# xiph/daala

Hardware: AMD Instinct MI355X
Metric: 1080p all-intra transform blocks/s (filter+DCT+PVQ) (higher is better)
Workload: dtype int32 (lifting DCT/filters) + f64 (PVQ search)

## Files before the change

### daala_amd/build.py

```python
import os
import subprocess
import sys
from concurrent.futures import ThreadPoolExecutor

HERE = os.path.dirname(os.path.abspath(__file__))
CSRC = os.path.join(HERE, "csrc")
LIBDIR = os.path.join(HERE, "lib")
LIB = os.path.join(LIBDIR, "libdaalahip.so")
EXP_LIB = os.path.join(LIBDIR, "libdaalahip_exp.so")
EXP_OBJDIR = os.path.join(LIBDIR, "exp")
HIPCC = os.environ.get("HIPCC", "/opt/rocm/bin/hipcc")
SOURCES = ["dct_kernels.hip", "lapped_kernels.hip", "pvq_kernels.hip", "pvq_bands.hip", "pvq_ref.hip", "pvq_refbands.hip", "image_kernels.hip", "dering_kernels.hip", "dering_cache.hip", "frame_cache.hip",
           "odhip_host.hip", "ctx.hip", "quant.hip", "pipeline.hip", "y4m.hip", "dist_kernels.hip", "rate_host.hip", "export_kernels.hip", "metrics_kernels.hip", "mc_kernels.hip"]
FLAGS = ["--offload-arch=gfx950", "-O3", "-std=c++17", "-fPIC",
         "-ffp-contract=off", "-fno-fast-math", "-Wall",
         "-Wno-unused-function"]


def _deps():
    out = []
    for root, _, files in os.walk(CSRC):
        for f in files:
            out.append(os.path.join(root, f))
    out.append(os.path.join(os.path.dirname(HERE), "include", "daala_hip.h"))
    return out


def _stale(target, deps):
    if not os.path.exists(target):
        return True
    t = os.path.getmtime(target)
    return any(os.path.getmtime(d) > t for d in deps)


def build(force=False, verbose=False, experiments=True):
    os.makedirs(LIBDIR, exist_ok=True)
    os.makedirs(EXP_OBJDIR, exist_ok=True)
    deps = _deps()
    variants = [(LIB, LIBDIR, [])]
    if experiments:
        variants.append((EXP_LIB, EXP_OBJDIR, ["-DODHIP_EXPERIMENTS"]))

    def run(cmd):
        if verbose:
            print(" ".join(cmd), flush=True)
        r = subprocess.run(cmd, capture_output=True, text=True)
        if r.returncode != 0:
            raise RuntimeError("hipcc failed:\n%s\n%s" % (" ".join(cmd), r.stderr))
        return r.stderr

    for lib, objdir, extra in variants:
        objs = []
        jobs = []
        for src in SOURCES:
            obj = os.path.join(objdir, src.replace(".hip", ".o"))
            objs.append(obj)
            if force or _stale(obj, deps):
                jobs.append([HIPCC] + FLAGS + extra + ["-c", os.path.join(CSRC, src), "-o", obj])
        try:
            with ThreadPoolExecutor(max_workers=min(8, os.cpu_count() or 4)) as ex:
                for warn in ex.map(run, jobs):
                    if verbose and warn:
                        print(warn)
            if jobs or force or _stale(lib, objs):
                run([HIPCC, "--offload-arch=gfx950", "-shared", "-fPIC", "-o", lib] + objs)
        except RuntimeError:
            if lib == LIB or experiments != "optional":
                raise
            print("daala_amd.build: the experiments variant failed to build (the product library is intact)",
                  file=sys.stderr)
    return LIB


def build_variant(name, extra_flags, verbose=False):
    outdir = os.path.join(HERE, "lib_" + name)
    os.makedirs(outdir, exist_ok=True)
    lib = os.path.join(outdir, "libdaalahip.so")
    stamp = os.path.join(outdir, "flags.txt")
    flags_changed = not os.path.exists(stamp) or open(stamp).read() != " ".join(extra_flags)
    deps = _deps()
    jobs = []
    objs = []
    for src in SOURCES:
        obj = os.path.join(outdir, src.replace(".hip", ".o"))
        objs.append(obj)
        if flags_changed or _stale(obj, deps):
            jobs.append([HIPCC] + FLAGS + list(extra_flags) + ["-c", os.path.join(CSRC, src), "-o", obj])

    def run(cmd):
        if verbose:
            print(" ".join(cmd), flush=True)
        r = subprocess.run(cmd, capture_output=True, text=True)
        if r.returncode != 0:
            raise RuntimeError("hipcc failed:\n%s\n%s" % (" ".join(cmd), r.stderr))

    with ThreadPoolExecutor(max_workers=min(8, os.cpu_count() or 4)) as ex:
        list(ex.map(run, jobs))
    if jobs or not os.path.exists(lib):
        run([HIPCC, "--offload-arch=gfx950", "-shared", "-fPIC", "-o", lib] + objs)
    with open(stamp, "w") as f:
        f.write(" ".join(extra_flags))
    return lib


if __name__ == "__main__":
    if "--variant" in sys.argv:
        i = sys.argv.index("--variant")
        print(build_variant(sys.argv[i + 1], sys.argv[i + 2:], verbose=True))
    else:
        print(build(force="--force" in sys.argv, verbose=True))
```

### daala_amd/csrc/od_sel.cuh

```cuda
#pragma once

namespace {

__device__ __forceinline__ unsigned long long od_cmp_gt(double a, double b) {
  unsigned long long m;
  asm("v_cmp_gt_f64_e64 %0, %1, %2" : "=s"(m) : "v"(a), "v"(b));
  return m;
}

__device__ __forceinline__ int od_sel(unsigned long long m, int t, int f) {
  int d;
  asm("v_cndmask_b32_e64 %0, %1, %2, %3" : "=v"(d) : "v"(f), "v"(t), "s"(m));
  return d;
}

__device__ __forceinline__ void od_inc(int &j) {
  asm("v_add_u32 %0, 1, %0" : "+v"(j));
}

__device__ __forceinline__ double od_cvt_u(int v) {
  double d;
  asm volatile("v_cvt_f64_u32_e32 %0, %1" : "=v"(d) : "v"(v));
  return d;
}

__device__ __forceinline__ double od_sel(unsigned long long m, double t, double f) {
  const int lo = od_sel(m, __double2loint(t), __double2loint(f));
  const int hi = od_sel(m, __double2hiint(t), __double2hiint(f));
  return __hiloint2double(hi, lo);
}

}
```

### daala_amd/csrc/pvq_refbands.hip

```cpp
#include "../../include/daala_hip.h"
#include <math.h>
#include <stdio.h>
#include <stdlib.h>
#include <string.h>
#include "od_ctx.cuh"
#include "od_pvq_math.cuh"
#include "od_occupancy.cuh"
#include "od_krange.cuh"
#include "od_band_stage.cuh"
#include "gen/od_scan_tables.h"
#define OD_RSQ_TABLE_N 512
#define OD_RSQ_HUGE
#include "pvq_search.cuh"
#include "pvq_row.cuh"
#include "pvq_regs.cuh"

namespace {

constexpr int kMaxJobs = 8;
constexpr int kMaxItems = kMaxJobs*ODHIP_MAX_BANDS;
constexpr int kSlots = ODHIP_PVQ_REF_SLOTS;
constexpr int kUncCap = 1 << 16;
constexpr double kDefaultMargin = 1e-9;

// ... 673 lines not shown
      int32_t tmp = odq_mult16_16(r16[e], proj_1);
      tmp = outshift >= 0 ? odq_shr_round(tmp, outshift) : odq_shl32(tmp, -outshift);
      const int16_t v = (int16_t)(x16[e] - tmp);
      if (live && i != m) xro[i - (i > m)] = v;
    }
  }
  if (live) {
    if constexpr (E == 8) {
      *reinterpret_cast<uint4 *>(x16o + l*E) = make_uint4(pack16(x16[0], x16[1]),
       pack16(x16[2], x16[3]), pack16(x16[4], x16[5]), pack16(x16[6], x16[7]));
      *reinterpret_cast<uint4 *>(r16o + l*E) = make_uint4(pack16(r16[0], r16[1]),
       pack16(r16[2], r16[3]), pack16(r16[4], r16[5]), pack16(r16[6], r16[7]));
    }
    else {
#pragma unroll
      for (int e = 0; e < E; e += 2) {
        *reinterpret_cast<uint32_t *>(x16o + l*E + e) = pack16(x16[e], x16[e + 1]);
        *reinterpret_cast<uint32_t *>(r16o + l*E + e) = pack16(r16[e], r16[e + 1]);
      }
    }
    if (l == 0) prep_write(it, rec + band, job, band, blk, xshift, rshift, p, r_null, flip, m, s);
  }
}


struct ItemPtr {
  int4 *head;
  int4 *tail;
  int4 *res;
  long stride;
};

__device__ __forceinline__ ItemPtr item_ptr(const RJob &jb, int band, long blk) {
  ItemPtr p;
  const long plane = (long)jb.nb_bands*kSlots*jb.nblocks;
  p.head = reinterpret_cast<int4 *>(jb.items) + (long)band*kSlots*jb.nblocks + blk;
  p.tail = p.head + plane;
  p.res = p.tail + plane;
  p.stride = jb.nblocks;
  return p;
}

__device__ __forceinline__ void refb_candidates(const RJob &jb, int band, long blk,
 int theta_override, int4 (*stage)[kWave]) {
  const int lane = threadIdx.x;
  odhip_pvq_refband *rp = jb.rec + blk*jb.nb_bands + band;
  odhip_pvq_refband r = *rp;
  if (theta_override >= 0) r.theta = theta_override;
  const int n = jb.off[band + 1] - jb.off[band];
  const int beta = jb.beta[band];
  const ItemPtr ip = item_ptr(jb, band, blk);
  int nitems = 0;
  int kmax_theta = 0;
  int kmax_noref = 0;
  if (r.flags & ODHIP_REFBAND_THETA) {
    const int gain_bound = (r.cg - r.gain_offset) >> ODQ_CGAIN_SHIFT;
    const double scale_1 = __ddiv_rn(1., kThetaScale);
    for (int i = gain_bound - 1 > 1 ? gain_bound - 1 : 1; i <= gain_bound + 1; i++) {
      const int32_t qcg = odq_shl32(i, ODQ_CGAIN_SHIFT) + r.gain_offset;
      const int ts = odq_pvq_compute_max_theta(qcg, beta);
      const double t = __ddiv_rn(((r.theta*scale_1)*2), kPi)*ts;
      int lower = (int)floor(.5 + t) - 2;
      if (lower < 0) lower = 0;
      int upper = (int)ceil(t);
      if (upper > ts - 1) upper = ts - 1;
      for (int j = lower; j <= upper && nitems < kSlots - 2; j++) {
        const int4 c = make_int4(i, j, ts, odq_compute_k_ref(j, n));
        kmax_theta = c.w > kmax_theta ? c.w : kmax_theta;
        int pos = nitems;
        while (pos > 0) {
          const int4 q = stage[pos - 1][lane];
          const int cmp = q.w == c.w ? q.x - c.x : q.w - c.w;
          if (cmp <= 0) break;
          stage[pos][lane] = q;
          pos--;
        }
        stage[pos][lane] = c;
        nitems++;
      }
    }
  }
  const int ntheta = nitems;
  int flags = r.flags & ~ODHIP_REFBAND_NOREF;
  if ((jb.is_keyframe && jb.pli == 0) || r.corr < .5 || r.cg < odq_shl32(2, ODQ_CGAIN_SHIFT)) {
    flags |= ODHIP_REFBAND_NOREF;
    const int gain_bound = r.cg >> ODQ_CGAIN_SHIFT;
    for (int i = gain_bound > 1 ? gain_bound : 1; i <= gain_bound + 1; i++) {
      const int kk = odq_compute_k_noref(odq_shl32(i, ODQ_CGAIN_SHIFT), n, beta);
      stage[nitems][lane] = make_int4(i, -1, 0, kk);
      kmax_noref = kk > kmax_noref ? kk : kmax_noref;
      nitems++;
    }
  }
  for (int i = 0; i < nitems; i++) ip.head[i*ip.stride] = stage[i][lane];
  int4 v;
  v.x = (int)((uint32_t)(uint16_t)r.m | (uint32_t)(uint8_t)r.s << 16 | (uint32_t)flags << 24);
  v.y = r.theta;
  v.z = nitems;
  v.w = ntheta;
  reinterpret_cast<int4 *>(rp)[2] = v;
  jb.keys[(long)band*jb.nblocks + blk] = (unsigned short)(kSortBins - 1 - od_work_bin(kmax_theta + kmax_noref));
}

__global__ __launch_bounds__(kWave) void k_refb_cands(RItems it) {
  const int item = find_item(it, blockIdx.x);
  const RJob &jb = it.jobs[it.job[item]];
  const long blk = (long)(blockIdx.x - it.wg_start[item])*kWave + threadIdx.x;
  __shared__ int4 stage[kSlots][kWave];
  if (blk >= jb.nblocks) return;
  refb_candidates(jb, it.band[item], blk, -1, stage);
}

__global__ __launch_bounds__(kWave) void k_refb_cands_list(const RJob *jobs, const Unc *list, int count) {
  __shared__ int4 stage[kSlots][kWave];
  const int i = blockIdx.x*kWave + threadIdx.x;
  if (i >= count) return;
  const Unc e = list[i];
  refb_candidates(jobs[e.job], e.band, e.blk, e.theta, stage);
}

struct RefBest {
  double best_cost;
  int chosen;
  int yslot;
  int noref;
  int32_t qtheta;
  int gain;
  int theta;
  int ts;
  int k;
  bool close;
};

struct NoDecide {
  template <class V>
  __device__ __forceinline__ void offer(int, bool, const int4 &, int32_t, int, double, int, const V &) {}
};

template <class V, class D>
__device__ __forceinline__ void refb_loops(const RJob &jb, int band, long blk, bool writer,
 bool may_store, double lambda, V &v, D &dec) {
  const odhip_pvq_refband r = jb.rec[blk*jb.nb_bands + band];
  const int off = jb.off[band];
  const int n = jb.off[band + 1] - off;
  const long nblocks = jb.nblocks;
  const int len = jb.len;
  int16_t *const yout = jb.y;
  const ItemPtr ip = item_ptr(jb, band, blk);
  const double s2 = (1./256)*(1./256);
  const double t1 = 1./32768;
  const int32_t cg = r.cg;
  const double dist0 = r.dist0;
  if (r.ntheta > 0) {
    v.load(jb.xr + blk*len + off, true);
    int prev_k = 0;
    int cur_slot = -1;
    int cur_mom = 0;
    double cos_dist = 0;
    const int32_t theta = r.theta;
    int4 hnext = ip.head[0];
    for (int idx = 0; idx < r.ntheta; idx++) {
      const int4 h = hnext;
      hnext = ip.head[(idx + 1 < r.nitems ? idx + 1 : idx)*ip.stride];
      const int32_t qcg = odq_shl32(h.x, ODQ_CGAIN_SHIFT) + r.gain_offset;
      const int32_t qtheta = odq_pvq_compute_theta(h.y, h.z);
      const int k = h.w;
      double dist_theta = 2 - (2.*odq_pvq_cos(theta - qtheta))*t1;
      double dist = (1.4*(qcg - cg))*(qcg - cg) + (qcg*(double)cg)*dist_theta;
      dist *= s2;
      if (dist > dist0 + 1.0*lambda && k != 0) {
        if (writer) ip.tail[idx*ip.stride] = make_int4(qcg, qtheta, ODHIP_REFITEM_WITH_REF, -1);
        continue;
      }
      if (k > ODHIP_PVQ_MAX_K) {
        if (writer) {
          atomicAdd(jb.krange, 1u);
          ip.tail[idx*ip.stride] = make_int4(qcg, qtheta, ODHIP_REFITEM_WITH_REF | ODHIP_REFITEM_K_RANGE,
           -1);
        }
        continue;
      }
      const double sin_prod = ((odq_pvq_sin(theta)*t1)*odq_pvq_sin(qtheta))*t1;
      if (k == 0) {
        cos_dist = 0;
        cur_slot = -1;
        cur_mom = 0;
      }
      else if (k != prev_k) {
        cos_dist = v.search(n - 1, k, prev_k, ((qcg*(double)cg)*sin_prod)*s2, lambda);
        cur_slot = idx;
        cur_mom = v.moment();
        if (may_store) v.store(yout + ((long)idx*nblocks + blk)*len + off);
      }
      prev_k = k;
      dist_theta = 2 - (2.*odq_pvq_cos(theta - qtheta))*t1 + sin_prod*(2 - 2*cos_dist);
      dist = (1.4*(qcg - cg))*(qcg - cg) + (qcg*(double)cg)*dist_theta;
      dist *= s2;
      if (writer) {
        ip.tail[idx*ip.stride] = make_int4(qcg, qtheta,
         ODHIP_REFITEM_WITH_REF | ODHIP_REFITEM_SEARCHED | cur_mom << ODHIP_REFITEM_MOMENT_SHIFT, cur_slot);
        ip.res[idx*ip.stride] = make_int4(__double2loint(cos_dist), __double2hiint(cos_dist),
         __double2loint(dist), __double2hiint(dist));
      }
      dec.offer(idx, true, h, qtheta, cur_slot, dist, cur_mom, v);
    }
  }
  if (r.nitems > r.ntheta) {
    v.load(jb.x16 + blk*len + off, false);
    int prev_k = 0;
    for (int idx = r.ntheta; idx < r.nitems; idx++) {
      const int4 h = ip.head[idx*ip.stride];
      const int32_t qcg = odq_shl32(h.x, ODQ_CGAIN_SHIFT);
      const int k = h.w;
      double dist = (1.4*(qcg - cg))*(qcg - cg);
      dist *= s2;
      if (dist > dist0 && k != 0) {
        if (writer) ip.tail[idx*ip.stride] = make_int4(qcg, 0, 0, -1);
        continue;
      }
      if (k > ODHIP_PVQ_MAX_K) {
        if (writer) atomicAdd(jb.krange, 1u);
        if (writer) ip.tail[idx*ip.stride] = make_int4(qcg, 0, ODHIP_REFITEM_K_RANGE, -1);
        continue;
      }
      const double cos_dist = v.search(n, k, prev_k, (qcg*(double)cg)*s2, lambda);
      prev_k = k;
      const int mom = v.moment();
      if (may_store) v.store(yout + ((long)idx*nblocks + blk)*len + off);
      dist = (1.4*(qcg - cg))*(qcg - cg) + (qcg*(double)cg)*(2 - 2*cos_dist);
      dist *= s2;
      if (writer) {
        ip.tail[idx*ip.stride] = make_int4(qcg, 0, ODHIP_REFITEM_SEARCHED | mom << ODHIP_REFITEM_MOMENT_SHIFT, idx);
        ip.res[idx*ip.stride] = make_int4(__double2loint(cos_dist), __double2hiint(cos_dist),
         __double2loint(dist), __double2hiint(dist));
      }
      dec.offer(idx, false, h, 0, idx, dist, mom, v);
    }
  }
}

struct LdsVector {
  short *xs;
  unsigned short *ys;
  int lane;
  int n;
  __device__ __forceinline__ void load(const int16_t *src, bool pad) {
    const int cnt = n - (pad ? 1 : 0);
    for (int j = 0; j < cnt; j++) xs[j*kWave + lane] = src[j];
  }
  __device__ __forceinline__ double search(int n_true, int k, int prev_k, double g2, double lambda) {
    double yy;
    cur = n_true;
    return od_pvq_search_lane(xs, ys, lane, n_true, k, prev_k, g2, lambda, &yy);
  }
  __device__ __forceinline__ void store(int16_t *dst) {
    for (int j = 0; j < cur; j++) {
      const int yj = ys[j*kWave + lane];
      dst[j] = (int16_t)(xs[j*kWave + lane] < 0 ? -yj : yj);
    }
  }
  __device__ __forceinline__ int moment() const {
    int m = 0;
    for (int j = 1; j < cur; j++) m += j*ys[j*kWave + lane];
    return m;
  }
  int cur;
};

#ifdef ODHIP_EXPERIMENTS
__global__ __launch_bounds__(kWave) void k_refb_search(RItems it) {
  extern __shared__ __attribute__((aligned(16))) unsigned short lds[];
  od_rsqrt_init(threadIdx.x);
  const int item = find_item(it, blockIdx.x);
  const RJob &jb = it.jobs[it.job[item]];
  const int band = it.band[item];
  const int n = jb.off[band + 1] - jb.off[band];
  const long pos = (long)(blockIdx.x - it.wg_start[item])*kWave + threadIdx.x;
  if (pos >= jb.nblocks) return;
  const long blk = jb.ids[(long)band*jb.nblocks + pos];
  LdsVector v = {(short *)lds, lds + n*kWave, (int)threadIdx.x, n, 0};
  NoDecide nd;
  refb_loops(jb, band, blk, true, true, it.lambda, v, nd);
}
#endif

__global__ __launch_bounds__(kWave) void k_refb_search_list(const RJob *jobs, const Unc *list, int count,
 double lambda) {
  extern __shared__ __attribute__((aligned(16))) unsigned short lds[];
  od_rsqrt_init(threadIdx.x);
  if (threadIdx.x != 0 || (int)blockIdx.x >= count) return;
  const Unc e = list[blockIdx.x];
  const RJob &jb = jobs[e.job];
  LdsVector v = {(short *)lds, lds + 128*kWave, 0, jb.off[e.band + 1] - jb.off[e.band], 0};
  NoDecide nd;
  refb_loops(jb, e.band, e.blk, true, true, lambda, v, nd);
}

__device__ __forceinline__ uint32_t pack_pulses(int s0, int y0, int s1, int y1) {
  return pack16(s0 ? -y0 : y0, s1 ? -y1 : y1);
}

template <int E, int G>
struct RowVector {
  int ax[E];
  unsigned sg;
  int y[E];
  int row;
  int l;
  int force;
  double xx;
  double norm_1;
  double cxy;
  double cyy;
  __device__ __forceinline__ void load(const int16_t *src, bool pad) {
    const int16_t *p = src + l*E;
    sg = 0;
#pragma unroll
    for (int e = 0; e < E; e++) {
      const int v = p[e];
      ax[e] = abs(v);
      sg |= (unsigned)(v < 0) << e;
      y[e] = 0;
    }
    if (pad && l == G - 1) {
      ax[E - 1] = 0;
      sg &= ~(1u << (E - 1));
    }
    od_row_norm<E, G>(ax, &xx, &norm_1);
  }
  __device__ __forceinline__ double search(int n_true, int k, int prev_k, double g2, double lambda) {
#ifdef ODHIP_EXPERIMENTS
    const int placed = prev_k > 0 && prev_k <= k ? prev_k : 0;
    const int greedy = k - (1 + k/4) - placed;
    pulses += greedy > 0 ? greedy : 0;
    rate_pulses += k - placed - (greedy > 0 ? greedy : 0);
    return od_pvq_search_row<E, G>(ax, y, row, l, n_true, k, prev_k, g2, lambda, force, xx, norm_1,
     &cxy, &cyy, &replays);
#else
    return od_pvq_search_row<E, G>(ax, y, row, l, n_true, k, prev_k, g2, lambda, force, xx, norm_1,
     &cxy, &cyy);
#endif
  }
#ifdef ODHIP_EXPERIMENTS
  int replays = 0;
  int pulses = 0;
  int rate_pulses = 0;
#endif
  __device__ __forceinline__ int moment() const {
    int m = 0;
#pragma unroll
    for (int e = 0; e < E; e++) m += (l*E + e)*y[e];
    return grp_sum<G>(m);
  }
  __device__ __forceinline__ void store(int16_t *dst) {
    int16_t *p = dst + l*E;
    if constexpr (E == 8) {
      *reinterpret_cast<uint4 *>(p) = make_uint4(pack_pulses(sg & 1, y[0], sg & 2, y[1]),
       pack_pulses(sg & 4, y[2], sg & 8, y[3]), pack_pulses(sg & 16, y[4], sg & 32, y[5]),
       pack_pulses(sg & 64, y[6], sg & 128, y[7]));
    }
    else {
#pragma unroll
      for (int e = 0; e < E; e += 2) {
        *reinterpret_cast<uint32_t *>(p + e) = pack_pulses(sg & (1u << e), y[e], sg & (2u << e), y[e + 1]);
      }
    }
  }
};

#ifdef ODHIP_EXPERIMENTS
__device__ unsigned long long gRowReplayStats[4];
#endif

template <int E, int G>
__global__ __launch_bounds__(kWave) void k_pvq_search_row(const int16_t *x_in, int n_true, const int32_t *k_in,
 od_coeff *y_out, const double *g2_in, double lambda, int force_scan, double *cos_out, int32_t *replays_out,
 long nbands) {
  constexpr int n = E*G;
  constexpr int C = kWave/G;
  od_rsqrt_init(threadIdx.x);
  const int lane = threadIdx.x;
  const int row = lane/G;
  const int l = lane%G;
  const long band = (long)blockIdx.x*C + row;
  const bool live = band < nbands;
  const long b = live ? band : nbands - 1;
  int ax[E];
  int y[E];
  unsigned sg = 0;
#pragma unroll
  for (int e = 0; e < E; e++) {
    const int j = l*E + e;
    const int v = j < n_true ? x_in[b*n_true + j] : 0;
    ax[e] = abs(v);
    sg |= (unsigned)(v < 0) << e;
    y[e] = 0;
  }
  double xx;
  double norm_1;
  od_row_norm<E, G>(ax, &xx, &norm_1);
  double cxy = 0;
  double cyy = 0;
  int replays = 0;
  int k = k_in[b];
  k = k < 0 ? 0 : k > 32767 ? 32767 : k;
  const double c = od_pvq_search_row<E, G>(ax, y, row, l, n_true, k, 0, g2_in[b], lambda, force_scan, xx, norm_1,
   &cxy, &cyy, &replays);
  if (live) {
#pragma unroll
    for (int e = 0; e < E; e++) {
      const int j = l*E + e;
      if (j < n_true) y_out[band*n_true + j] = sg >> e & 1 ? -y[e] : y[e];
    }
    if (l == 0) {
      cos_out[band] = c;
      if (replays_out) replays_out[band] = replays;
    }
  }
  (void)n;
}

template <int E, int G>
__global__ __launch_bounds__(kWave) __attribute__((amdgpu_waves_per_eu(3, 3))) void k_refb_search_row(RItems it) {
  od_rsqrt_init(threadIdx.x);
  const int item = find_item(it, blockIdx.x);
  const RJob &jb = it.jobs[it.job[item]];
  const int lane = threadIdx.x;
  RowVector<E, G> v;
  v.row = lane/G;
  v.l = lane%G;
  v.force = it.perturb >> 1;
  const long nblocks = jb.nblocks;
  const long pos = (long)(blockIdx.x - it.wg_start[item])*(kWave/G) + v.row;
  const bool live = pos < nblocks;
  const long blk = jb.ids[(long)it.band[item]*nblocks + (live ? pos : nblocks - 1)];
  NoDecide nd;
  refb_loops(jb, it.band[item], blk, live && v.l == 0, live, it.lambda, v, nd);
}

template <int N>
struct RegVector {
  static constexpr int SH = N == 15 ? 1 : 0;
  int ax[N];
  unsigned sg;
  int y[N];
  double xx;
  double norm_1;
  double cxy;
  double cyy;
  __device__ __forceinline__ void load(const int16_t *src, bool pad) {
    const uint4 *p = reinterpret_cast<const uint4 *>(src - SH);
    sg = 0;
    uint32_t w[(N + SH)/2];
#pragma unroll
    for (int q = 0; q < (N + SH)/8; q++) {
      const uint4 t = p[q];
      w[4*q] = t.x;
      w[4*q + 1] = t.y;
      w[4*q + 2] = t.z;
      w[4*q + 3] = t.w;
    }
#pragma unroll
    for (int i = 0; i < N; i++) {
      const int t = (int16_t)(w[(i + SH) >> 1] >> (16*((i + SH) & 1)));
      ax[i] = abs(t);
      sg |= (unsigned)(t < 0) << i;
      y[i] = 0;
    }
    if (pad) {
      ax[N - 1] = 0;
      sg &= ~(1u << (N - 1));
    }
    od_regs_norm<N>(ax, &xx, &norm_1);
  }
  __device__ __forceinline__ double search(int n_true, int k, int prev_k, double g2, double lambda) {
    return od_pvq_search_regs<N>(ax, y, n_true, k, prev_k, g2, lambda, xx, norm_1, &cxy, &cyy);
  }
  __device__ __forceinline__ int moment() const {
    int m = 0;
#pragma unroll
    for (int i = 1; i < N; i++) m += i*y[i];
    return m;
  }
  __device__ __forceinline__ void store(int16_t *dst) {
    uint4 *p = reinterpret_cast<uint4 *>(dst - SH);
    int t[N + SH];
    if (SH) t[0] = 0;
#pragma unroll
    for (int i = 0; i < N; i++) t[i + SH] = (sg >> i) & 1 ? -y[i] : y[i];
#pragma unroll
    for (int q = 0; q < (N + SH)/8; q++) {
      p[q] = make_uint4(pack16(t[8*q], t[8*q + 1]), pack16(t[8*q + 2], t[8*q + 3]),
       pack16(t[8*q + 4], t[8*q + 5]), pack16(t[8*q + 6], t[8*q + 7]));
    }
  }
};



__device__ __forceinline__ int neg_interleave(int x, int ref) {
  if (x < ref) return -2*(x - ref) - 1;
  if (x < 2*ref) return 2*(x - ref);
  return x - 1;
}

__device__ unsigned char gRBandOf[OD_SCAN_LEN];

template <int N, class YGet>
__device__ __forceinline__ void refb_finish(const RItems &it, int job, const RJob &jb, int band, long blk,
 const odhip_pvq_refband &r, const RefBest &best, YGet yget);

template <int N, int PRICE>
__device__ __forceinline__ void refb_choose_band(const RItems &it, int job, const RJob &jb, int band,
 long blk, const double *given) {
  constexpr int SH = N == 15 ? 1 : 0;
  constexpr int NW = (N + SH)/2;
  const long bi = blk*jb.nb_bands + band;
  const odhip_pvq_refband r = jb.rec[bi];
  const ItemPtr ip = item_ptr(jb, band, blk);
  const double *rate = PRICE == 2 ? given : PRICE == 0 && jb.rate ? jb.rate + bi*(kSlots + 1) : nullptr;
  const double lambda = it.lambda;
  const int off = jb.off[band];
  double best_cost = r.dist0 + lambda*(rate ? rate[0] : 0.);
  bool close = false;
  int noref = jb.is_keyframe ? 1 : 0;
  int32_t best_qtheta = 0;
  int chosen = -1;
  int yslot = -1;
  int4 tails[kSlots];
  int dlo[kSlots];
  int dhi[kSlots];
#pragma unroll
  for (int idx = 0; idx < kSlots; idx++) {
    tails[idx] = make_int4(0, 0, 0, -1);
    dlo[idx] = 0;
    dhi[idx] = 0;
    if (idx < r.nitems) {
      tails[idx] = ip.tail[idx*ip.stride];
      const int4 res = ip.res[idx*ip.stride];
      dlo[idx] = res.z;
      dhi[idx] = res.w;
    }
  }
#pragma unroll
  for (int idx = 0; idx < kSlots; idx++) {
    if (idx >= r.nitems) continue;
    const int4 tail = tails[idx];
    if (!(tail.z & ODHIP_REFITEM_SEARCHED)) continue;
    double cost = __hiloint2double(dhi[idx], dlo[idx]);
    if (PRICE == 1) {
      const int4 hd = ip.head[idx*ip.stride];
      const bool with_ref = idx < r.ntheta;
      const int sum = (int)((unsigned)tail.z >> ODHIP_REFITEM_MOMENT_SHIFT);
      cost = cost + lambda*odq_pvq_rate_fast(sum, hd.w, N, hd.x, with_ref ? r.icgr : 0, with_ref ? hd.y : -1,
       with_ref ? hd.z : 0, jb.is_keyframe, jb.pli);
      const double d = cost - best_cost;
      if ((d < 0 ? -d : d) <= it.tol_scale*odq_rate_tol(cost, best_cost)) close = true;
    }
    else cost = cost + lambda*(rate ? rate[1 + idx] : 0.);
    if (idx < r.ntheta ? cost < best_cost : cost <= best_cost) {
      best_cost = cost;
      chosen = idx;
      yslot = tail.w;
      if (idx < r.ntheta) {
        best_qtheta = tail.y;
        noref = 0;
      }
      else noref = 1;
    }
  }
  RefBest best;
  best.best_cost = best_cost;
  best.chosen = chosen;
  best.yslot = yslot;
  best.noref = noref;
  best.qtheta = best_qtheta;
  best.gain = best.theta = best.ts = best.k = 0;
  best.close = PRICE == 1 && close;
  if (chosen >= 0) {
    const int4 head = ip.head[chosen*ip.stride];
    best.gain = head.x;
    best.theta = head.y;
    best.ts = head.z;
    best.k = head.w;
  }
  uint32_t yw[NW];
  if (yslot >= 0) {
    const uint4 *yp = reinterpret_cast<const uint4 *>(jb.y + ((long)yslot*jb.nblocks + blk)*jb.len
     + off - SH);
    if constexpr (NW >= 4) {
#pragma unroll
      for (int v = 0; v < NW/4; v++) {
        const uint4 q = yp[v];
        yw[4*v] = q.x;
        yw[4*v + 1] = q.y;
        yw[4*v + 2] = q.z;
        yw[4*v + 3] = q.w;
      }
    }
  }
  else {
#pragma unroll
    for (int v = 0; v < NW; v++) yw[v] = 0;
  }
  refb_finish<N>(it, job, jb, band, blk, r, best,
   [&](int i) -> int { return (int16_t)(yw[(i + SH) >> 1] >> (16*((i + SH) & 1))); });
}

template <int N, class YGet>
__device__ __forceinline__ void refb_finish(const RItems &it, int job, const RJob &jb, int band, long blk,
 const odhip_pvq_refband &r, const RefBest &best, YGet yget) {
  constexpr int SH = N == 15 ? 1 : 0;
  constexpr int NW = (N + SH)/2;
  const long bi = blk*jb.nb_bands + band;
  const int off = jb.off[band];
  const int cfl_enabled = jb.is_keyframe && jb.pli != 0;
  const int chosen = best.chosen;
  const int yslot = best.yslot;
  const int noref = best.noref;
  const int32_t best_qtheta = best.qtheta;
  int qg = 0;
  int itheta = jb.is_keyframe ? -1 : 0;
  int max_theta = 0;
  int best_k = 0;
  if (best.close) {
    const unsigned slot = atomicAdd(it.pcount, 1u);
    if (slot < (unsigned)kPUncCap) {
      PUncR *e = it.plist + slot;
      e->job = job;
      e->band = band;
      e->blk = (unsigned)blk;
    }
  }
  if (chosen >= 0) {
    qg = best.gain;
    best_k = best.k;
    if (noref) {
      itheta = -1;
      max_theta = 0;
    }
    else {
      itheta = best.theta;
      max_theta = best.ts;
    }
  }
  int skip = 0;
  if (noref) {
    if (qg == 0) skip = 1;
  }
  else {
    if (!jb.is_keyframe && qg == 0) skip = r.icgr ? 1 : 2;
    if (qg == r.icgr && itheta == 0 && !cfl_enabled) skip = 2;
  }
  int4 *ch = reinterpret_cast<int4 *>(jb.choice + bi*16);
  ch[0] = make_int4(chosen, qg, noref, itheta);
  ch[1] = make_int4(max_theta, best_k, skip, jb.is_keyframe ? (noref ? qg : neg_interleave(qg, r.icgr))
   : (noref ? qg - 1 : neg_interleave(qg + 1, r.icgr + 1)));
  if (skip) {
    const int flip = (r.flags & ODHIP_REFBAND_FLIP) != 0;
    ch[2] = make_int4(skip == 2 ? (flip ? 4 : 1) : 0, -1, 0, 0);
    ch[3] = make_int4(0, 0, 0, 0);
    return;
  }
  const int32_t g = odq_gain_expand(odq_shl32(qg, ODQ_CGAIN_SHIFT) + (noref ? 0 : r.gain_offset),
   job_q(jb, band, blk), jb.beta[band]);
  const int nn = N - (!noref);
  int yy = 0;
#pragma unroll
  for (int i = 0; i < N; i++) {
    const int v = i < nn ? yget(i) : 0;
    yy += v*v;
  }
  int gshift = odq_ilog(g) - 14;
  gshift = gshift > 0 ? gshift : 0;
  int32_t scale = 0;
  if (yy != 0) {
    int rsqrt_shift;
    const int16_t rsqrt = odq_rsqrt(yy, &rsqrt_shift);
    scale = odq_vshr_round(rsqrt*(int64_t)g, rsqrt_shift + gshift - 16);
  }
  const int qshift = ODQ_QM_INV_SHIFT - gshift;
  if (noref) {
    ch[2] = make_int4(2, yslot, scale, qshift);
    ch[3] = make_int4(0, 0, 0, 0);
    return;
  }
  const int m = r.m;
  const int s = r.s;
  scale = (int32_t)floor(.5 + (scale*(1./32768))*odq_pvq_sin(best_qtheta));
  const int16_t xm = (int16_t)floor(.5 + ((-s*odq_shr_round(g, gshift))*(1./32768))*odq_pvq_cos(best_qtheta));
  uint32_t rw[NW];
  {
    const uint4 *rp = reinterpret_cast<const uint4 *>(jb.r16 + blk*jb.len + off - SH);
#pragma unroll
    for (int v = 0; v < NW/4; v++) {
      const uint4 q = rp[v];
      rw[4*v] = q.x;
// ... 1499 lines not shown
```

### daala_amd/csrc/pvq_row.cuh

```cuda
#pragma once
#include <type_traits>
#include "od_sel.cuh"

namespace {

template <int G>
__device__ __forceinline__ int grp_sum(int v) {
  v += row_mov<OD_DPP_XOR1>(v);
  v += row_mov<OD_DPP_XOR2>(v);
  if (G == 16) {
    v += row_mov<OD_DPP_HALF_MIRROR>(v);
    v += row_mov<OD_DPP_MIRROR>(v);
  }
  return v;
}

template <int G>
__device__ __forceinline__ double grp_sum(double v) {
  v += row_mov<OD_DPP_XOR1>(v);
  v += row_mov<OD_DPP_XOR2>(v);
  if (G == 16) {
    v += row_mov<OD_DPP_HALF_MIRROR>(v);
    v += row_mov<OD_DPP_MIRROR>(v);
  }
  return v;
}

template <int G>
__device__ __forceinline__ int grp_min(int v) {
  v = min(v, row_mov<OD_DPP_XOR1>(v));
  v = min(v, row_mov<OD_DPP_XOR2>(v));
  if (G == 16) {
    v = min(v, row_mov<OD_DPP_HALF_MIRROR>(v));
    v = min(v, row_mov<OD_DPP_MIRROR>(v));
  }
  return v;
}

template <int G>
__device__ __forceinline__ int grp_max(int v) {
  v = max(v, row_mov<OD_DPP_XOR1>(v));
  v = max(v, row_mov<OD_DPP_XOR2>(v));
  if (G == 16) {
    v = max(v, row_mov<OD_DPP_HALF_MIRROR>(v));
    v = max(v, row_mov<OD_DPP_MIRROR>(v));
  }
  return v;
}

template <int G>
__device__ __forceinline__ float grp_max(float v) {
  v = fmaxf(v, __int_as_float(row_mov<OD_DPP_XOR1>(__float_as_int(v))));
  v = fmaxf(v, __int_as_float(row_mov<OD_DPP_XOR2>(__float_as_int(v))));
  if (G == 16) {
    v = fmaxf(v, __int_as_float(row_mov<OD_DPP_HALF_MIRROR>(__float_as_int(v))));
    v = fmaxf(v, __int_as_float(row_mov<OD_DPP_MIRROR>(__float_as_int(v))));
  }
  return v;
}

template <int G>
__device__ __forceinline__ unsigned grp_ballot(bool p, int grp) {
  const unsigned long long m = __ballot(p);
  return (unsigned)(m >> (G*grp)) & ((1u << G) - 1u);
}

template <int G>
__device__ __forceinline__ int grp_bcast(int v, int grp, int src) {
  return __shfl(v, G*grp + src, 64);
}

template <int G>
__device__ __forceinline__ double grp_bcast(double v, int grp, int src) {
  return __shfl(v, G*grp + src, 64);
}

__device__ __forceinline__ double row_sum(double v) { return grp_sum<16>(v); }
__device__ __forceinline__ int row_max(int v) { return grp_max<16>(v); }

template <int E, int G>
__device__ __forceinline__ void od_row_norm(const int (&ax)[E], double *xx_out, double *norm_1_out) {
  double xx = 0;
#pragma unroll
  for (int e = 0; e < E; e++) xx += (double)ax[e]*(double)ax[e];
  xx = grp_sum<G>(xx);
  *xx_out = xx;
  *norm_1_out = __ddiv_rn(1., __dsqrt_rn(1e-30 + xx));
}

template <int E, int G>
__device__ __forceinline__ double od_pvq_search_row(const int (&ax)[E], int (&y)[E], int row,
 int l, int n_true, int k, int prev_k, double g2, double pvq_norm_lambda, int force_scan,
 double xx, double norm_1, double *cxy, double *cyy, int *replays = nullptr) {
  constexpr int n = G*E;
  static_assert(E > 1, "the single-precision screen folds from candidate 0 of each lane, which must not be the PAD");
  static_assert(G == 4 || G == 16, "a quad or a DPP row");
  const bool pad_lane = n_true != n && l == G - 1;
  const double lambda = __ddiv_rn(pvq_norm_lambda, 1e-30 + g2);
  double xy = 0;
  double yy = 0;
  int i = 0;
  const bool chained = prev_k > 0 && prev_k <= k;
  if (chained) {
  }
  else if (k > 2) {
    double l1 = 0;
#pragma unroll
    for (int e = 0; e < E; e++) l1 += (double)ax[e];
    l1 = grp_sum<G>(l1);
    const double l1_inv = __ddiv_rn(1., l1 > 1e-100 ? l1 : 1e-100);
#pragma unroll
    for (int e = 0; e < E; e++) {
      const double tmp = (k*(double)ax[e])*l1_inv;
      const int v = (int)floor(tmp);
      y[e] = v > 0 ? v : 0;
      xy += (double)ax[e]*y[e];
      yy += (double)(y[e]*y[e]);
      i += y[e];
    }
  }
  else {
#pragma unroll
    for (int e = 0; e < E; e++) y[e] = 0;
  }
  if (chained) {
    xy = *cxy;
    yy = *cyy;
    i = prev_k;
  }
  else {
    xy = grp_sum<G>(xy);
    yy = grp_sum<G>(yy);
    i = grp_sum<G>(i);
  }
  const int rdo_pulses = 1 + k/4;
  const int n_greedy = k - rdo_pulses;
  const double delta_rate = n_true == n ? 3./n : 3./(n - 1);
  while (__any(i < n_greedy)) {
    const bool on = i < n_greedy;
    const int yyp1 = (int)yy + 1;
    const float xyf = (float)xy;
    float af[E];
    float bf[E];
    int bi[E];
    float baf = 0;
    float bbf = 1;
    int bax = 0;
    int bbi = 1;
#pragma unroll
    for (int e = 0; e < E; e++) {
      const float tf = xyf + (float)ax[e];
      af[e] = tf*tf;
      bi[e] = yyp1 + 2*y[e];
      bf[e] = (float)bi[e];
      if (e == E - 1 && pad_lane) af[e] = -1.f;
      if (e == 0 || af[e]*bbf > baf*bf[e]) {
        baf = af[e];
        bbf = bf[e];
        bax = ax[e];
        bbi = bi[e];
      }
    }
    const int key = __float_as_int(baf*__builtin_amdgcn_rcpf(bbf));
    const int kmax = grp_max<G>(key);
    const unsigned wmask = grp_ballot<G>(key == kmax, row);
    const int wl = wmask ? __ffs(wmask) - 1 : 0;
    const int wx = grp_bcast<G>(bax, row, wl);
    const int wbi = grp_bcast<G>(bbi, row, wl);
    const float thr = __int_as_float(kmax)*(1.f - 7.62939453125e-06f);
    bool bad = force_scan != 0 || wmask == 0;
    int first_dup = n;
#pragma unroll
    for (int e = E - 1; e >= 0; e--) {
      bool dup = (ax[e] == wx) & (bi[e] == wbi);
      if (e == E - 1 && pad_lane) dup = false;
      const bool loses = af[e] < bf[e]*thr;
      first_dup = dup ? l*E + e : first_dup;
      bad |= !(dup | loses);
    }
    int pos;
    int px = wx;
    double nb = (double)wbi;
    if (grp_ballot<G>(bad && on, row) != 0) {
      if (replays) ++*replays;
      double sa = 0;
      double sb = 1;
      int sx = 0;
      pos = 0;
#pragma unroll 1
      for (int j = 0; j < n; j++) {
        const int e = j % E;
        int cx = ax[0];
        int cy = y[0];
#pragma unroll
        for (int t = 1; t < E; t++) {
          if (e == t) {
            cx = ax[t];
            cy = y[t];
          }
        }
        cx = grp_bcast<G>(cx, row, j/E);
        cy = grp_bcast<G>(cy, row, j/E);
        const double tt = xy + od_cvt_u(cx);
        double ca = tt*tt;
        const double cb = (double)(yyp1 + 2*cy);
        if (n_true != n && j == n - 1) ca = -1;
        if (j == 0 || ca*sb > sa*cb) {
          sa = ca;
          sb = cb;
          sx = cx;
          pos = j;
        }
      }
      nb = sb;
      px = sx;
    }
    else pos = grp_min<G>(first_dup);
#pragma unroll
    for (int e = 0; e < E; e++) {
      if (on && l*E + e == pos) y[e]++;
    }
    if (on) {
      xy = xy + (double)px;
      yy = nb;
      i++;
    }
  }
  double pen[E];
#pragma unroll
  for (int e = 0; e < E; e++) pen[e] = (lambda*(l*E + e))*delta_rate;
  const double norm2 = 2*norm_1;
  while (__any(i < k)) {
    const bool on = i < k;
    const int yyi = (int)yy;
    double bc = 0;
    int bi = 0;
    auto scan = [&](auto fast) {
#pragma unroll
      for (int e = 0; e < E; e++) {
        const int j = l*E + e;
        double tmp_xy = xy + od_cvt_u(ax[e]);
        const int idx = yyi + 2*y[e] + 1;
        const double r = decltype(fast)::value ? od_rsq_lds[(idx < OD_RSQ_TABLE_N ? idx : OD_RSQ_TABLE_N) - 1]
         : od_rsqrt_table(idx);
        tmp_xy = (tmp_xy*norm2)*r - pen[e];
        if (e == E - 1 && pad_lane) tmp_xy = -1.7976931348623157e308;
        if (e == 0 || tmp_xy > bc) {
          bc = tmp_xy;
          bi = j;
        }
      }
    };
    if (!__any(on && yyi + 2*i + 1 > OD_RSQ_TABLE_N)) scan(std::true_type());
    else scan(std::false_type());
    double bm = bc;
    bm = fmax(bm, row_mov<OD_DPP_XOR1>(bm));
    bm = fmax(bm, row_mov<OD_DPP_XOR2>(bm));
    if (G == 16) {
      bm = fmax(bm, row_mov<OD_DPP_HALF_MIRROR>(bm));
      bm = fmax(bm, row_mov<OD_DPP_MIRROR>(bm));
    }
    const unsigned tmask = grp_ballot<G>(bc == bm, row);
    bi = grp_bcast<G>(bi, row, tmask ? __ffs(tmask) - 1 : 0);
    const int pos = bi;
    int px = 0;
    int py = 0;
#pragma unroll
    for (int e = 0; e < E; e++) {
      if (on && l*E + e == pos) {
        px = ax[e];
        py = y[e];
        y[e]++;
      }
    }
    px = grp_bcast<G>(px, row, pos/E);
    py = grp_bcast<G>(py, row, pos/E);
    if (on) {
      xy = xy + (double)px;
      yy = yy + (double)(2*py) + 1;
      i++;
    }
  }
  *cxy = xy;
  *cyy = yy;
  return __ddiv_rn(xy, 1e-100 + __dsqrt_rn(xx*yy));
}

}
```

Before: 1.180 billion.

## Store PVQ row magnitudes as floats and pack greedy screen into float2 pairs

The row-level PVQ search now keeps coefficient magnitudes as floats instead of ints, so the single-precision greedy screen needs no per-step int-to-float conversion. It evaluates candidates two at a time with packed float2 math and a tree fold. The y increment is rewritten as a branchless compare-add. The build also adds a register gate that fails compilation if the lean row kernels exceed 168 VGPRs or spill, which risks build breakage but guards occupancy.

```diff
diff --git a/daala_amd/build.py b/daala_amd/build.py
--- a/daala_amd/build.py
+++ b/daala_amd/build.py
@@ -1,4 +1,5 @@
 import os
+import re
 import subprocess
 import sys
 from concurrent.futures import ThreadPoolExecutor
@@ -15,6 +16,38 @@
 FLAGS = ["--offload-arch=gfx950", "-O3", "-std=c++17", "-fPIC",
          "-ffp-contract=off", "-fno-fast-math", "-Wall",
          "-Wno-unused-function"]
+GATE_SOURCE = "pvq_refbands.hip"
+GATE_FLAG = "-Rpass-analysis=kernel-resource-usage"
+GATE_KERNELS = ["k_refb_lean_rowILi8ELi16E", "k_refb_lean_rowILi8ELi4E"]
+GATE_VGPRS = 168
+
+
+def check_register_gate(report):
+    found = {}
+    name = None
+    for line in report.splitlines():
+        m = re.search(r"remark: Function Name: (\S+)", line)
+        if m:
+            name = next((k for k in GATE_KERNELS if k in m.group(1)), None)
+            if name:
+                found.setdefault(name, [None, None])
+            continue
+        if name is None:
+            continue
+        m = re.search(r"remark:\s+VGPRs: (\d+)", line)
+        if m:
+            found[name][0] = int(m.group(1))
+        m = re.search(r"remark:\s+ScratchSize \[bytes/lane\]: (\d+)", line)
+        if m:
+            found[name][1] = int(m.group(1))
+    for k in GATE_KERNELS:
+        if k not in found or None in found[k]:
+            raise RuntimeError("register gate: no resource report for %s" % k)
+        vgprs, scratch = found[k]
+        if vgprs > GATE_VGPRS or scratch != 0:
+            raise RuntimeError("register gate: %s uses %d VGPRs and %d bytes of scratch per lane (limit %d and 0)"
+                               % (k, vgprs, scratch, GATE_VGPRS))
+    return {k: tuple(v) for k, v in found.items()}
 
 
 def _deps():
@@ -47,6 +80,9 @@
         r = subprocess.run(cmd, capture_output=True, text=True)
         if r.returncode != 0:
             raise RuntimeError("hipcc failed:\n%s\n%s" % (" ".join(cmd), r.stderr))
+        if GATE_FLAG in cmd:
+            check_register_gate(r.stderr)
+            return ""
         return r.stderr
 
     for lib, objdir, extra in variants:
@@ -56,7 +92,8 @@
             obj = os.path.join(objdir, src.replace(".hip", ".o"))
             objs.append(obj)
             if force or _stale(obj, deps):
-                jobs.append([HIPCC] + FLAGS + extra + ["-c", os.path.join(CSRC, src), "-o", obj])
+                gate = [GATE_FLAG] if src == GATE_SOURCE and lib == LIB else []
+                jobs.append([HIPCC] + FLAGS + extra + gate + ["-c", os.path.join(CSRC, src), "-o", obj])
         try:
             with ThreadPoolExecutor(max_workers=min(8, os.cpu_count() or 4)) as ex:
                 for warn in ex.map(run, jobs):
diff --git a/daala_amd/csrc/od_sel.cuh b/daala_amd/csrc/od_sel.cuh
--- a/daala_amd/csrc/od_sel.cuh
+++ b/daala_amd/csrc/od_sel.cuh
@@ -24,6 +24,12 @@
   return d;
 }
 
+__device__ __forceinline__ double od_cvt_f(float v) {
+  double d;
+  asm volatile("v_cvt_f64_f32_e32 %0, %1" : "=v"(d) : "v"(v));
+  return d;
+}
+
 __device__ __forceinline__ double od_sel(unsigned long long m, double t, double f) {
   const int lo = od_sel(m, __double2loint(t), __double2loint(f));
   const int hi = od_sel(m, __double2hiint(t), __double2hiint(f));
diff --git a/daala_amd/csrc/pvq_refbands.hip b/daala_amd/csrc/pvq_refbands.hip
--- a/daala_amd/csrc/pvq_refbands.hip
+++ b/daala_amd/csrc/pvq_refbands.hip
@@ -999,7 +999,7 @@
 
 template <int E, int G>
 struct RowVector {
-  int ax[E];
+  float ax[E];
   unsigned sg;
   int y[E];
   int row;
@@ -1015,7 +1015,7 @@
 #pragma unroll
     for (int e = 0; e < E; e++) {
       const int v = p[e];
-      ax[e] = abs(v);
+      ax[e] = (float)abs(v);
       sg |= (unsigned)(v < 0) << e;
       y[e] = 0;
     }
@@ -1082,14 +1082,14 @@
   const long band = (long)blockIdx.x*C + row;
   const bool live = band < nbands;
   const long b = live ? band : nbands - 1;
-  int ax[E];
+  float ax[E];
   int y[E];
   unsigned sg = 0;
 #pragma unroll
   for (int e = 0; e < E; e++) {
     const int j = l*E + e;
     const int v = j < n_true ? x_in[b*n_true + j] : 0;
-    ax[e] = abs(v);
+    ax[e] = (float)abs(v);
     sg |= (unsigned)(v < 0) << e;
     y[e] = 0;
   }
diff --git a/daala_amd/csrc/pvq_row.cuh b/daala_amd/csrc/pvq_row.cuh
--- a/daala_amd/csrc/pvq_row.cuh
+++ b/daala_amd/csrc/pvq_row.cuh
@@ -4,6 +4,35 @@
 
 namespace {
 
+typedef float od_f2 __attribute__((ext_vector_type(2)));
+
+struct Cand {
+  float a;
+  float b;
+  float x;
+  int y;
+};
+
+template <int E, int P0, int NP>
+__device__ __forceinline__ Cand od_fold_pairs(const od_f2 (&a2)[E/2], const od_f2 (&bs)[E/2], const float (&ax)[E],
+ const int (&y)[E]) {
+  Cand lo;
+  Cand up;
+  od_f2 pr;
+  if constexpr (NP == 1) {
+    lo = Cand{a2[P0].x, bs[P0].y, ax[2*P0], y[2*P0]};
+    up = Cand{a2[P0].y, bs[P0].x, ax[2*P0 + 1], y[2*P0 + 1]};
+    pr = a2[P0]*bs[P0];
+  }
+  else {
+    lo = od_fold_pairs<E, P0, NP/2>(a2, bs, ax, y);
+    up = od_fold_pairs<E, P0 + NP/2, NP/2>(a2, bs, ax, y);
+    pr = od_f2{lo.a, up.a}*od_f2{up.b, lo.b};
+  }
+  const bool take = pr.y > pr.x;
+  return Cand{take ? up.a : lo.a, take ? up.b : lo.b, take ? up.x : lo.x, take ? up.y : lo.y};
+}
+
 template <int G>
 __device__ __forceinline__ int grp_sum(int v) {
   v += row_mov<OD_DPP_XOR1>(v);
@@ -79,20 +108,23 @@
 __device__ __forceinline__ int row_max(int v) { return grp_max<16>(v); }
 
 template <int E, int G>
-__device__ __forceinline__ void od_row_norm(const int (&ax)[E], double *xx_out, double *norm_1_out) {
+__device__ __forceinline__ void od_row_norm(const float (&ax)[E], double *xx_out, double *norm_1_out) {
   double xx = 0;
 #pragma unroll
-  for (int e = 0; e < E; e++) xx += (double)ax[e]*(double)ax[e];
+  for (int e = 0; e < E; e++) { const double d = od_cvt_f(ax[e]); xx += d*d; }
   xx = grp_sum<G>(xx);
   *xx_out = xx;
   *norm_1_out = __ddiv_rn(1., __dsqrt_rn(1e-30 + xx));
 }
 
 template <int E, int G>
-__device__ __forceinline__ double od_pvq_search_row(const int (&ax)[E], int (&y)[E], int row,
+__device__ __forceinline__ double od_pvq_search_row(const float (&ax_in)[E], int (&y)[E], int row,
  int l, int n_true, int k, int prev_k, double g2, double pvq_norm_lambda, int force_scan,
  double xx, double norm_1, double *cxy, double *cyy, int *replays = nullptr) {
   constexpr int n = G*E;
+  float ax[E];
+#pragma unroll
+  for (int e = 0; e < E; e++) ax[e] = ax_in[e];
   static_assert(E > 1, "the single-precision screen folds from candidate 0 of each lane, which must not be the PAD");
   static_assert(G == 4 || G == 16, "a quad or a DPP row");
   const bool pad_lane = n_true != n && l == G - 1;
@@ -106,15 +138,15 @@
   else if (k > 2) {
     double l1 = 0;
 #pragma unroll
-    for (int e = 0; e < E; e++) l1 += (double)ax[e];
+    for (int e = 0; e < E; e++) l1 += od_cvt_f(ax[e]);
     l1 = grp_sum<G>(l1);
     const double l1_inv = __ddiv_rn(1., l1 > 1e-100 ? l1 : 1e-100);
 #pragma unroll
     for (int e = 0; e < E; e++) {
-      const double tmp = (k*(double)ax[e])*l1_inv;
+      const double tmp = (k*od_cvt_f(ax[e]))*l1_inv;
       const int v = (int)floor(tmp);
       y[e] = v > 0 ? v : 0;
-      xy += (double)ax[e]*y[e];
+      xy += od_cvt_f(ax[e])*y[e];
       yy += (double)(y[e]*y[e]);
       i += y[e];
     }
@@ -140,68 +172,66 @@
     const bool on = i < n_greedy;
     const int yyp1 = (int)yy + 1;
     const float xyf = (float)xy;
-    float af[E];
-    float bf[E];
-    int bi[E];
-    float baf = 0;
-    float bbf = 1;
-    int bax = 0;
-    int bbi = 1;
-#pragma unroll
-    for (int e = 0; e < E; e++) {
-      const float tf = xyf + (float)ax[e];
-      af[e] = tf*tf;
-      bi[e] = yyp1 + 2*y[e];
-      bf[e] = (float)bi[e];
-      if (e == E - 1 && pad_lane) af[e] = -1.f;
-      if (e == 0 || af[e]*bbf > baf*bf[e]) {
-        baf = af[e];
-        bbf = bf[e];
-        bax = ax[e];
-        bbi = bi[e];
-      }
-    }
-    const int key = __float_as_int(baf*__builtin_amdgcn_rcpf(bbf));
+    const od_f2 xy2 = {xyf, xyf};
+    od_f2 a2[E/2];
+    od_f2 bs[E/2];
+#pragma unroll
+    for (int p = 0; p < E/2; p++) {
+      const od_f2 x2 = {ax[2*p], ax[2*p + 1]};
+      const od_f2 t2 = xy2 + x2;
+      a2[p] = t2*t2;
+      bs[p] = od_f2{(float)(yyp1 + 2*y[2*p + 1]), (float)(yyp1 + 2*y[2*p])};
+    }
+    if (pad_lane) a2[E/2 - 1].y = -1.f;
+    const Cand w = od_fold_pairs<E, 0, E/2>(a2, bs, ax, y);
+    const int key = __float_as_int(w.a*__builtin_amdgcn_rcpf(w.b));
     const int kmax = grp_max<G>(key);
     const unsigned wmask = grp_ballot<G>(key == kmax, row);
     const int wl = wmask ? __ffs(wmask) - 1 : 0;
-    const int wx = grp_bcast<G>(bax, row, wl);
-    const int wbi = grp_bcast<G>(bbi, row, wl);
+    const int wx = grp_bcast<G>(__float_as_int(w.x), row, wl);
+    const int wy = grp_bcast<G>(w.y, row, wl);
     const float thr = __int_as_float(kmax)*(1.f - 7.62939453125e-06f);
+    const od_f2 thr2 = {thr, thr};
     bool bad = force_scan != 0 || wmask == 0;
-    int first_dup = n;
-#pragma unroll
-    for (int e = E - 1; e >= 0; e--) {
-      bool dup = (ax[e] == wx) & (bi[e] == wbi);
-      if (e == E - 1 && pad_lane) dup = false;
-      const bool loses = af[e] < bf[e]*thr;
-      first_dup = dup ? l*E + e : first_dup;
-      bad |= !(dup | loses);
-    }
+    int fd = n;
+#pragma unroll
+    for (int p = E/2 - 1; p >= 0; p--) {
+      const od_f2 lim = bs[p]*thr2;
+#pragma unroll
+      for (int h = 1; h >= 0; h--) {
+        const int e = 2*p + h;
+        bool dup = (__float_as_int(ax[e]) == wx) & (y[e] == wy);
+        if (e == E - 1 && pad_lane) dup = false;
+        const bool loses = (h ? a2[p].y < lim.x : a2[p].x < lim.y);
+        fd = dup ? e : fd;
+        bad |= !(dup | loses);
+      }
+    }
+    const int first_dup = l*E + fd;
     int pos;
-    int px = wx;
-    double nb = (double)wbi;
+    float px = __int_as_float(wx);
+    double nb = (double)(yyp1 + 2*wy);
     if (grp_ballot<G>(bad && on, row) != 0) {
       if (replays) ++*replays;
       double sa = 0;
       double sb = 1;
-      int sx = 0;
+      float sx = 0;
       pos = 0;
 #pragma unroll 1
       for (int j = 0; j < n; j++) {
         const int e = j % E;
-        int cx = ax[0];
+        int cxb = __float_as_int(ax[0]);
         int cy = y[0];
 #pragma unroll
         for (int t = 1; t < E; t++) {
           if (e == t) {
-            cx = ax[t];
+            cxb = __float_as_int(ax[t]);
             cy = y[t];
           }
         }
-        cx = grp_bcast<G>(cx, row, j/E);
+        const float cx = __int_as_float(grp_bcast<G>(cxb, row, j/E));
         cy = grp_bcast<G>(cy, row, j/E);
-        const double tt = xy + od_cvt_u(cx);
+        const double tt = xy + od_cvt_f(cx);
         double ca = tt*tt;
         const double cb = (double)(yyp1 + 2*cy);
         if (n_true != n && j == n - 1) ca = -1;
@@ -216,10 +246,10 @@
       px = sx;
     }
     else pos = grp_min<G>(first_dup);
-#pragma unroll
-    for (int e = 0; e < E; e++) {
-      if (on && l*E + e == pos) y[e]++;
-    }
+    int rel = on ? pos - l*E : -1;
+    asm("" : "+v"(rel));
+#pragma unroll
+    for (int e = 0; e < E; e++) y[e] += (int)(rel == e);
     if (on) {
       xy = xy + (double)px;
       yy = nb;
@@ -239,7 +269,7 @@
 #pragma unroll
       for (int e = 0; e < E; e++) {
         const int j = l*E + e;
-        double tmp_xy = xy + od_cvt_u(ax[e]);
+        double tmp_xy = xy + od_cvt_f(ax[e]);
         const int idx = yyi + 2*y[e] + 1;
         const double r = decltype(fast)::value ? od_rsq_lds[(idx < OD_RSQ_TABLE_N ? idx : OD_RSQ_TABLE_N) - 1]
          : od_rsqrt_table(idx);
@@ -268,7 +298,7 @@
 #pragma unroll
     for (int e = 0; e < E; e++) {
       if (on && l*E + e == pos) {
-        px = ax[e];
+        px = __float_as_int(ax[e]);
         py = y[e];
         y[e]++;
       }
@@ -276,7 +306,7 @@
     px = grp_bcast<G>(px, row, pos/E);
     py = grp_bcast<G>(py, row, pos/E);
     if (on) {
-      xy = xy + (double)px;
+      xy = xy + (double)__int_as_float(px);
       yy = yy + (double)(2*py) + 1;
       i++;
     }
```

Result: no change. 1.182 billion (median of 6 runs) (+0.2%).
